# Blackgaurd/pathtracer-cpp

Hardware: AMD Instinct MI355X
Metric: Mray/s (all bounces) + achieved HBM GB/s, Cornell 1024² 10k spp depth-5 (higher is better)
Workload: dtype f32

## Files before the change

### include/pt_hip_debug.h

```cpp
#ifndef PT_HIP_DEBUG_H
#define PT_HIP_DEBUG_H

#include "pt_hip.h"

#ifdef __cplusplus
extern "C" {
#endif

int pt_debug_math(int device, int which, const float* in, int n, float* out);
int pt_debug_sweep(int device, int which, uint32_t lo_bits, uint32_t hi_bits, uint64_t* mismatches,
                   uint32_t* first_bad);
int pt_debug_rgb8(int device, const float* linear_rgb, int32_t res_x, int32_t res_y, float gamma, uint8_t* rgb8);
int pt_debug_rccl_failover(int32_t n_devices, int32_t fail_step, int64_t* out);
int pt_debug_wide_verify(const pt_scene* scene, int32_t width);
int pt_debug_pack_hash(const pt_scene* scene, uint64_t* hash);
int pt_rtc_check(const pt_scene* scene, char* src_out, size_t cap);
int pt_debug_rtc_start(const pt_scene* scene);
int64_t pt_debug_rtc_cache(int32_t op);

int pt_debug_ctx_flags(const pt_ctx* ctx, int32_t out[5]);
int pt_debug_ctx_plan(const pt_ctx* ctx, int64_t out[24]);
int pt_debug_walk_placement(int32_t num_nodes, int32_t num_tris, int32_t tree_depth, int32_t tri_f4,
                            int32_t rec_rows, uint64_t lds_usable, int32_t out[4]);
int pt_debug_scene_dark(const pt_scene* scene);
int pt_debug_emit_reject(const float* box6, const float* org, const float* dir, int64_t n, uint8_t* out);
int pt_debug_emit_slab_reject(const float* box6, const float* org, const float* inv, int64_t n, uint8_t* out);
int pt_debug_emit_box(const pt_scene* scene, float out[6]);
int pt_debug_ctx_emit_reject(const pt_ctx* ctx, int32_t* on, float box[6], uint64_t* early);
int pt_debug_ray_stack(int32_t which, int32_t count, int32_t n, int32_t reserve, int32_t flag);
int pt_debug_flat_lds(int32_t num_tris, int32_t box_tab_bytes, int32_t pair_queue, int32_t rec_size, uint32_t out[10]);
int64_t pt_debug_counter(int32_t which);

#ifdef __cplusplus
}
#endif
#endif
```

### pathtracer-cpp_amd/csrc/pt_kernel.hip

```cpp
#include <hip/hip_runtime.h>

#include <stdint.h>
#include <stdio.h>
#include <stdlib.h>
#include <string.h>

#include <algorithm>
#include <chrono>
#include <future>
#include <map>
#include <memory>
#include <mutex>
#include <string>
#include <thread>
#include <vector>

#include <atomic>

#include "pt_grad.h"
#include "pt_hip_debug.h"
#include "pt_launch.h"
#include "pt_moments.h"
#include "pt_nee_grad.h"
#include "pt_rtc.h"
// ... 176 lines not shown

__global__ void pt_math_kernel(int which, const float* __restrict__ in, float* __restrict__ out, int n) {
    const int i = blockIdx.x * blockDim.x + threadIdx.x;
    if (i >= n) return;
    if (which == 0) {
        out[i] = acosf_ref(in[i]);
    } else if (which == 1) {
        float sv, cv;
        sincosf_ref(in[i], sv, cv);
        out[2 * i] = sv;
        out[2 * i + 1] = cv;
    } else if (which == 2) {
        const float* a = in + 9 * (size_t)i;
        Lcg g{__float_as_uint(a[0])};
        const int type = __float_as_int(a[1]);
        const v3 dd{a[3], a[4], a[5]}, nn{a[6], a[7], a[8]};
        v3 r;
        if (type == PT_MAT_SPECULAR) specular_dir(g, dd, nn, a[2], kMaxSpecularIters, r);
        else r = hemisphere_dir(g, nn);
        out[4 * i] = r.x;
        out[4 * i + 1] = r.y;
        out[4 * i + 2] = r.z;
        out[4 * i + 3] = __uint_as_float(g.s);
    }
}

__global__ void pt_sweep_kernel(int which, uint32_t lo, unsigned long long n, unsigned long long* bad,
                                uint32_t* first) {
    unsigned long long nb = 0;
    uint32_t fb = 0xffffffffu;
    const unsigned long long stride = (unsigned long long)gridDim.x * blockDim.x;
    for (unsigned long long i = (unsigned long long)blockIdx.x * blockDim.x + threadIdx.x; i < n; i += stride) {
        const uint32_t bits = lo + (uint32_t)i;
        const float x = __uint_as_float(bits);
        if (x != x) continue;
        bool same;
        if (which == 0) {
            same = __float_as_uint(rcp_exact(x)) == __float_as_uint(1.0f / x);
        } else if (which == 1) {
            same = __float_as_uint(sqrt_exact(x)) == __float_as_uint(__builtin_sqrtf(x));
        } else if (which == 4) {
            const float ax = __builtin_fabsf(x);
            if (!(ax >= 0x1p-60f && ax <= 0x1p60f)) continue;
            const uint32_t hsh = pt_mix32(bits * 0x9e3779b9u + 0x7f4a7c15u);
            const uint32_t e = (bits & 1u) ? 67u + (hsh >> 23) % 121u : 127u + (hsh >> 23) % 11u;
            const float b = __uint_as_float((e << 23) | (hsh & 0x7fffffu));
// ... 2290 lines not shown
    const EmitBox e = scene_emit_box(ps, scene_dark(ps));
    for (int a = 0; a < 3; a++) out[a] = e.lo[a], out[3 + a] = e.hi[a];
    return e.on ? 1 : 0;
}

int pt_debug_emit_reject(const float* box6, const float* org, const float* dir, int64_t n, uint8_t* out) {
    if (!box6 || !org || !dir || !out || n < 0) return set_error(PT_E_ARG, "pt_debug_emit_reject: bad argument");
    for (int64_t i = 0; i < n; i++) {
        const float *b = box6 + 6 * i, *o = org + 3 * i, *d = dir + 3 * i;
        out[i] = emit_reject(v3{b[0], b[1], b[2]}, v3{b[3], b[4], b[5]}, v3{o[0], o[1], o[2]}, v3{d[0], d[1], d[2]}) ? 1 : 0;
    }
    return PT_OK;
}

int pt_debug_emit_slab_reject(const float* box6, const float* org, const float* inv, int64_t n, uint8_t* out) {
    if (!box6 || !org || !inv || !out || n < 0) return set_error(PT_E_ARG, "pt_debug_emit_slab_reject: bad argument");
    for (int64_t i = 0; i < n; i++) {
        const float *b = box6 + 6 * i, *o = org + 3 * i, *v = inv + 3 * i;
        out[i] = emit_slab_reject(v3{b[0], b[1], b[2]}, v3{b[3], b[4], b[5]}, v3{o[0], o[1], o[2]}, v3{v[0], v[1], v[2]}) ? 1 : 0;
    }
    return PT_OK;
}

int pt_debug_ray_stack(int32_t which, int32_t count, int32_t n, int32_t reserve, int32_t flag) {
    switch (which) {
        case 0: return ray_stack_generate(count, n, reserve, flag != 0) ? 1 : 0;
        case 1: return ray_stack_filled(count, n);
        case 2: return ray_stack_dry(count, n) ? 1 : 0;
        case 3: return ray_stack_slot(count, n);
        case 4: return ray_stack_taken(count, n);
        case 5: return ray_stack_done(flag != 0, count, n != 0) ? 1 : 0;
    }
    return set_error(PT_E_ARG, "pt_debug_ray_stack: which = %d", which);
}

int pt_debug_flat_lds(int32_t num_tris, int32_t box_tab_bytes, int32_t pair_queue, int32_t rec_size, uint32_t out[10]) {
    if (!out || num_tris < 0 || box_tab_bytes < 0 || pair_queue < 0 || rec_size < 0)
        return set_error(PT_E_ARG, "pt_debug_flat_lds: bad argument");
    const FlatLds l = flat_lds_layout(3u * (unsigned)num_tris, 2u * (unsigned)num_tris, (unsigned)box_tab_bytes,
                                      (unsigned)pair_queue, (unsigned)rec_size);
    const uint32_t v[10] = {l.tris, l.mats, l.next_ray, l.best, l.next_at, l.boxtab, l.queues, l.rec_tri, l.rec_cos, l.bytes};
    memcpy(out, v, sizeof(v));
    return PT_OK;
}

int pt_debug_ctx_plan(const pt_ctx* c, int64_t out[24]) {
// ... 67 lines not shown
```

### pathtracer-cpp_amd/csrc/pt_math.h

```cpp
#pragma once

#if !defined(__HIPCC_RTC__)
#include <stdint.h>
#endif

#if defined(__HIPCC__)
#define PT_HD __host__ __device__ __forceinline__
#else
#define PT_HD inline
#endif

namespace pt {

PT_HD uint32_t f2u(float f) { return __builtin_bit_cast(uint32_t, f); }
PT_HD float u2f(uint32_t u) { return __builtin_bit_cast(float, u); }

struct v3 {
    float x, y, z;
};
PT_HD v3 mk(float x, float y, float z) { return v3{x, y, z}; }
PT_HD v3 add(v3 a, v3 b) { return v3{a.x + b.x, a.y + b.y, a.z + b.z}; }
PT_HD v3 sub(v3 a, v3 b) { return v3{a.x - b.x, a.y - b.y, a.z - b.z}; }
PT_HD v3 mul(v3 a, v3 b) { return v3{a.x * b.x, a.y * b.y, a.z * b.z}; }
PT_HD v3 scale(v3 a, float s) { return v3{a.x * s, a.y * s, a.z * s}; }
// ... 65 lines not shown
    if (__builtin_expect(out, 0)) return __builtin_sqrtf(x);
    return sqrt_fixup(x);
#endif
#else
    return __builtin_sqrtf(x);
#endif
}

template <bool kUnit = false>
PT_HD v3 rcp3_exact(v3 d, bool live = true) {
#if defined(__HIP_DEVICE_COMPILE__) && PT_WAVE_GUARD
    const float ax = __builtin_fabsf(d.x), ay = __builtin_fabsf(d.y), az = __builtin_fabsf(d.z);
    bool out = !(__builtin_fminf(__builtin_fminf(ax, ay), az) >= 0x1p-126f);
    if (!kUnit) out = out || !(__builtin_fmaxf(__builtin_fmaxf(ax, ay), az) <= 0x1p126f);
    v3 r{rcp_newton(d.x), rcp_newton(d.y), rcp_newton(d.z)};
    if (__builtin_expect(wave_any(live && out), 0)) r = v3{1.0f / d.x, 1.0f / d.y, 1.0f / d.z};
    return r;
#else
    (void)live;
    return v3{rcp_exact(d.x), rcp_exact(d.y), rcp_exact(d.z)};
#endif
}

PT_HD v3 normalize(v3 a) {
    float len = sqrt_exact(dot(a, a));
    return v3{a.x / len, a.y / len, a.z / len};
}

PT_HD float div_by_rcp(float a, float b, float y) {
#if defined(__HIP_DEVICE_COMPILE__)
    const float q0 = a * y;
    return __builtin_fmaf(__builtin_fmaf(-b, q0, a), y, q0);
#else
    (void)y;
    return a / b;
#endif
}

PT_HD v3 normalize_fast(v3 a) {
#if defined(__HIP_DEVICE_COMPILE__) && PT_WAVE_GUARD
    const float l2 = dot(a, a);
    const float mn = __builtin_fminf(__builtin_fminf(__builtin_fabsf(a.x), __builtin_fabsf(a.y)), __builtin_fabsf(a.z));
    const bool out = !(l2 >= 0x1p-100f && l2 <= 0x1p100f && mn >= 0x1p-60f);
    const float lf = sqrt_fixup(l2), y = rcp_newton(lf);
    v3 r{div_by_rcp(a.x, lf, y), div_by_rcp(a.y, lf, y), div_by_rcp(a.z, lf, y)};
    if (__builtin_expect(wave_any(out), 0)) {
// ... 48 lines not shown
    float t1x = (lb.x - o.x) * inv.x, t1y = (lb.y - o.y) * inv.y, t1z = (lb.z - o.z) * inv.z;
    float t2x = (rt.x - o.x) * inv.x, t2y = (rt.y - o.y) * inv.y, t2z = (rt.z - o.z) * inv.z;
    float tmax = __builtin_fminf(__builtin_fminf(__builtin_fmaxf(t1x, t2x), __builtin_fmaxf(t1y, t2y)),
                                 __builtin_fmaxf(t1z, t2z));
    float tmin = __builtin_fmaxf(__builtin_fmaxf(__builtin_fminf(t1x, t2x), __builtin_fminf(t1y, t2y)),
                                 __builtin_fminf(t1z, t2z));
    return __builtin_fmaxf(tmin, 0.0f) <= tmax;
}

PT_HD bool all_finite(v3 a) {
    return __builtin_fabsf(a.x) < __builtin_inff() && __builtin_fabsf(a.y) < __builtin_inff() &&
           __builtin_fabsf(a.z) < __builtin_inff();
}

PT_HD int emit_reject_axis(float lo, float hi, float o, float d) {
    return (int)(__builtin_fabsf(d) < 2.0f) & (((int)(o < lo) & (int)(d < 0.0f)) | ((int)(o > hi) & (int)(d > 0.0f)));
}
PT_HD bool emit_reject(v3 elb, v3 ert, v3 o, v3 d) {
    return (emit_reject_axis(elb.x, ert.x, o.x, d.x) | emit_reject_axis(elb.y, ert.y, o.y, d.y) |
            emit_reject_axis(elb.z, ert.z, o.z, d.z)) != 0;
}

PT_HD bool finite_nonzero(float x) { return ((int)(__builtin_fabsf(x) < __builtin_inff()) & (int)(x != 0.0f)) != 0; }
PT_HD bool emit_slab_reject_nonempty(v3 elb, v3 ert, v3 o, v3 inv, bool behind_only = false) {
    const int guard = (int)finite_nonzero(inv.x) & (int)finite_nonzero(inv.y) & (int)finite_nonzero(inv.z) &
                      (int)(__builtin_fabsf(o.x) < __builtin_inff()) & (int)(__builtin_fabsf(o.y) < __builtin_inff()) &
                      (int)(__builtin_fabsf(o.z) < __builtin_inff());
    const float t1x = (elb.x - o.x) * inv.x, t1y = (elb.y - o.y) * inv.y, t1z = (elb.z - o.z) * inv.z;
    const float t2x = (ert.x - o.x) * inv.x, t2y = (ert.y - o.y) * inv.y, t2z = (ert.z - o.z) * inv.z;
    const float tmax = __builtin_fminf(__builtin_fminf(__builtin_fmaxf(t1x, t2x), __builtin_fmaxf(t1y, t2y)),
                                       __builtin_fmaxf(t1z, t2z));
    const float tmin = __builtin_fmaxf(__builtin_fmaxf(__builtin_fminf(t1x, t2x), __builtin_fminf(t1y, t2y)),
                                       __builtin_fminf(t1z, t2z));
    return (guard & ((int)(tmax < 0.0f) | ((int)!behind_only & (int)(tmin > tmax)))) != 0;
}
PT_HD bool emit_box_empty(v3 elb, v3 ert) {
    return ((int)(elb.x > ert.x) | (int)(elb.y > ert.y) | (int)(elb.z > ert.z)) != 0;
}
PT_HD bool emit_slab_reject(v3 elb, v3 ert, v3 o, v3 inv) {
    return emit_box_empty(elb, ert) ? true : emit_slab_reject_nonempty(elb, ert, o, inv);
}

PT_HD bool tri_hit(v3 v1, v3 e1, v3 e2, v3 o, v3 d, float& t) {
    v3 h = cross(d, e2);
    float a = dot(e1, h);
    if (__builtin_fabsf(a) < 0x1.0c6f7cp-20f) return false;
    float f = rcp_exact(a);
    v3 s = sub(o, v1);
    float u = f * dot(s, h);
    if (u < 0.0f || u > 1.0f) return false;
    v3 q = cross(s, e1);
    float v = f * dot(d, q);
    if (v < 0.0f || u + v > 1.0f) return false;
    t = f * dot(e2, q);
    return t > 0.0f;
}

PT_HD bool tri_hit_nb(v3 v1, v3 e1, v3 e2, v3 o, v3 d, float& t) {
    v3 h = cross(d, e2);
    float a = dot(e1, h);
    const bool ok = !(__builtin_fabsf(a) < 0x1.0c6f7cp-20f);
#if defined(__HIP_DEVICE_COMPILE__)
    const float r = __builtin_amdgcn_rcpf(a);
// ... 232 lines not shown
```

### pathtracer-cpp_amd/csrc/pt_rtc.hip

```cpp
#include <hip/hip_runtime.h>
#include <hip/hiprtc.h>

#include <dlfcn.h>
#include <errno.h>
#include <fcntl.h>
#include <link.h>
#include <signal.h>
#include <spawn.h>
#include <stdint.h>
#include <stdio.h>
#include <stdlib.h>
#include <string.h>
#include <sys/socket.h>
#include <sys/stat.h>
#include <sys/wait.h>
#include <unistd.h>

#include <algorithm>
#include <atomic>
#include <chrono>
#include <fstream>
#include <future>
#include <limits>
#include <map>
// ... 210 lines not shown
            chain += std::string("        ") + w + " = shl1_add_bit(" + w + ", __builtin_amdgcn_ballot_w64(b" +
                     std::to_string(u) + "));\n";
        }
        acc = "#if KBOX\n        uint32_t lo, hi;\n" + chain + "#else\n" + acc + "#endif\n";
    }
    acc += "        const unsigned long long m = ((unsigned long long)hi << 32) | lo;\n";
    const bool single = leaves_single(leaves, n);
    const bool sign = tri_fast;
    std::string tabs = "{";
    for (size_t u = 0; u < box_tab.size(); u++) tabs += (u ? ", " : "") + std::to_string(box_tab[u]) + "u";
    tabs += box_tab.empty() ? "0u}" : "}";
    std::string rej = "    using EmitRej = NoEmitReject;\n";
    if (emit.on)
        rej = "    struct EmitRej {\n        static constexpr bool kCompiled = true;\n"
              "        __device__ __forceinline__ static bool on() { return true; }\n"
              "        __device__ __forceinline__ static bool rejected(v3 o, v3 d) {\n"
              "            return emit_reject(v3{" + litf(emit.lo[0]) + ", " + litf(emit.lo[1]) + ", " + litf(emit.lo[2]) +
              "}, v3{" + litf(emit.hi[0]) + ", " + litf(emit.hi[1]) + ", " + litf(emit.hi[2]) + "}, o, d);\n"
              "        }\n"
              "        static constexpr bool kSlab = !PT_EMIT_SIGN_ONLY;\n"
              "        __device__ __forceinline__ static bool rejected_slab(v3 o, v3, v3 inv) {\n"
              "            return emit_slab_reject(v3{" + litf(emit.lo[0]) + ", " + litf(emit.lo[1]) + ", " + litf(emit.lo[2]) +
              "}, v3{" + litf(emit.hi[0]) + ", " + litf(emit.hi[1]) + ", " + litf(emit.hi[2]) + "}, o, inv);\n"
              "        }\n    };\n";
    return std::string("#ifndef PT_FLAT_SIGN_MASK\n#define PT_FLAT_SIGN_MASK 0\n#endif\n#define KSIGN (PT_FLAT_SIGN_MASK && ") +
           (sign ? "1" : "0") + ")\n" + "#define KBOX " + (nbox > 0 ? "(!KSIGN)" : "0") + "\n" +
           "namespace pt {\nstruct SceneBoxMask {\n    static constexpr bool kSignMask = KSIGN;\n"
           "    static constexpr bool kBoxPairs = KBOX;\n    static constexpr bool kCamInvGen = PT_CAM_INV == 2;\n"
           "    static constexpr bool kRayStack = PT_RAY_STACK != 0;\n"
           "    static constexpr int kBoxes = " + std::to_string(nbox) +
           ";\n    static constexpr uint16_t kBoxTab[" + std::to_string(std::max<size_t>(1, box_tab.size())) + "] = " + tabs +
           ";\n    static constexpr bool kMask32 = " +
           (n <= 32 ? "true" : "false") + ";\n    static constexpr bool kSingleTri = " + (single ? "true" : "false") +
           ";\n    static constexpr bool kSpecular = " + (specular ? "true" : "false") +
           ";\n    static constexpr bool kTriFast = " + (tri_fast ? "true" : "false") +
           ";\n    static constexpr bool kAlbedoX2 = " + (albedo_x2 ? "true" : "false") +
           ";\n    static constexpr bool kDarkKnown = true;\n    static constexpr bool kDark = " + (dark ? "true" : "false") +
           ";\n    static constexpr bool kBaked = PT_KCONST != 0;\n    static constexpr int kNumTri4 = " +
           std::to_string(baked.num_tri4) + ", kNumMat4 = " + std::to_string(baked.num_mat4) +
           ", kBoxTabBytes = " + std::to_string(baked.box_tab_bytes) + ", kThetaLanes = " + std::to_string(baked.theta_lanes) +
           ";\n    static constexpr bool kPairs = " + (baked.pairs ? "true" : "false") +
           ";\n" + rej + "    __device__ __forceinline__ static unsigned long long "
           "mask(const TraceArgs&, v3 o, v3 inv) {\n" +
           body + tests + acc + "        return m;\n    }\n};\n}  // namespace pt\n";
}

struct RtcCache {
    std::mutex mu;
    std::map<std::string, RtcFuture> code;
    std::map<std::pair<int, std::string>, hipFunction_t> funcs;
    std::set<std::string> refused;
};
// ... 560 lines not shown
```

### pathtracer-cpp_amd/csrc/pt_trace.h

```cpp
#pragma once

#include "pt_hip.h"
#include "pt_math.h"
#include "pt_flatlds.h"
#include "pt_raystack.h"

namespace pt {

constexpr int kBlock = 256;
constexpr int kWave = 64;
static_assert(kRaySlots == kWave, "one prefetched camera ray per lane (pt_raystack.h)");
constexpr int kMaxSpecularIters = 1 << 16;
#ifndef PT_CHUNK
#define PT_CHUNK 1024
#endif
constexpr int kChunk = PT_CHUNK;
static_assert(kChunk >= kWave, "a work-pool refill must cover one claim of every lane of a wave");
constexpr int kMaxFlatLeaves = 64;

#ifndef PT_WAVES
#define PT_WAVES 7
#endif

#ifdef PT_STAMPS
// ... 301 lines not shown
constexpr int kEmitSlab = 1, kEmitSignOnly = 2, kEmitSlabEmpty = 3;
#ifndef PT_EMIT_SIGN_ONLY
#define PT_EMIT_SIGN_ONLY 0
#endif
struct KernargEmitSlabReject : KernargEmitReject {
    static constexpr bool kSlab = true;
    __device__ __forceinline__ static bool rejected_slab(v3 o, v3, v3 inv) {
        const auto* K = kernarg_args();
        const int mode = K->emit_on;
        if (mode == kEmitSlabEmpty) return true;
        return emit_slab_reject_nonempty(v3{K->emit_lo_x, K->emit_lo_y, K->emit_lo_z},
                                         v3{K->emit_hi_x, K->emit_hi_y, K->emit_hi_z}, o, inv, mode == kEmitSignOnly);
    }
};
template <typename Rej, typename = void>
struct RejSlab {
    static constexpr bool value = false;
};
template <typename Rej>
struct RejSlab<Rej, decltype((void)Rej::kSlab)> {
    static constexpr bool value = Rej::kCompiled && Rej::kSlab;
};

struct NodeBox {
    v3 lb, rt;
    int a, b;
};

__device__ __forceinline__ NodeBox load_node(const float4* __restrict__ nodes, int n) {
    const float4 p = nodes[2 * n], q = nodes[2 * n + 1];
    return NodeBox{v3{p.x, p.y, p.z}, v3{p.w, q.x, q.y}, __float_as_int(q.z), __float_as_int(q.w)};
}

template <bool kFiniteInv>
__device__ __forceinline__ bool box_hit(v3 lb, v3 rt, v3 o, v3 inv) {
    return kFiniteInv ? slab_hit_finite(lb, rt, o, inv) : slab_hit(lb, rt, o, inv);
}

template <bool kFiniteInv, typename NodePtr, typename TriPtr>
__device__ __forceinline__ int intersect_tree(NodePtr nodes, TriPtr tris, int* __restrict__ stk, int tid, v3 o,
                                              v3 d, v3 inv, float& t_out) {
    int hit = -1;
    float t = 1e30f;
    int sp = 0;
    const NodeBox root = load_node(nodes, 0);
    int ca = root.a, cb = root.b;
// ... 1138 lines not shown

#ifndef PT_CAM_KERNARG
#define PT_CAM_KERNARG 1
#endif
__device__ __forceinline__ void camera_ray(const TraceArgs& A, int q, int s, Lcg& g, v3& o, v3& d) {
    const auto* K = PT_CAM_KERNARG ? kernarg_args() : nullptr;
    const TraceArgs& C = PT_CAM_KERNARG ? *(const TraceArgs*)K : A;
    const int r = (int)fdiv((uint32_t)q, C.div_w);
    const int px = q - r * C.W;
    const int py = part_row(C, r);
    g.s = pt_sample_seed((uint32_t)(py * C.W + px), (uint32_t)s, C.seed);
    const float jy = g.next01();
    const float jx = g.next01();
    const float cx = ((float)px + jx) * C.cell - C.half_vres_x;
    const float cy = ((float)py + jy) * C.cell - C.half_vres_y;
    d = normalize_fast(v3{cx * C.col0_x + cy * C.col0_y + C.cz_col0, cx * C.col1_x + cy * C.col1_y + C.cz_col1,
                     cx * C.col2_x + cy * C.col2_y + C.cz_col2});
    o = v3{C.pos_x, C.pos_y, C.pos_z};
}

constexpr int kShadeGo = 0, kShadeEnd = 1, kShadeEndEarly = 2;

template <bool kSpecular = true, typename RecT = int, bool kIds = false, typename Rej = NoEmitReject,
          typename KC = ArgConsts>
__device__ __forceinline__ int shade_inv(const TraceArgs& A, const float4* __restrict__ mats,
                                          const float4* __restrict__ tris, RecT* __restrict__ rec_tri,
                                          float* __restrict__ rec_cos, int tid, int hit, float t, Lcg& g, v3& o,
                                          v3& d, v3& inv, int& k, v3& L, const KC& kc = KC()) {
    L = v3{0.0f, 0.0f, 0.0f};
    if (hit < 0) return kShadeEnd;
#ifdef PT_EXP_DUP_SHADE
    {
        int h2 = hit;
        asm volatile("" : "+v"(h2));
        const float4 tn2 = kIds ? tris[h2] : tris[3 * h2 + 2];
        const int row2 = kIds ? __float_as_int(tn2.w) : h2;
        const float4 m02 = mats[2 * row2], m12 = mats[2 * row2 + 1];
        v3 n2 = kIds ? v3{tn2.x, tn2.y, tn2.z} : v3{tn2.y, tn2.z, tn2.w};
        if (!(dot(n2, d) < 0.0f)) n2 = neg(n2);
        const v3 hp2 = add(o, scale(d, t));
        asm volatile("" ::"v"(m02.x), "v"(m12.x), "v"(hp2.x), "v"(hp2.y), "v"(hp2.z), "v"(n2.x), "v"(n2.y), "v"(n2.z));
    }
#endif
    float4 tn;
    int row = hit;
    if constexpr (kIds) {
        tn = tris[hit];
        row = __float_as_int(tn.w);
    }
    const float4 m0 = mats[2 * row], m1 = mats[2 * row + 1];
    const int type = __float_as_int(m0.x);
// ... 48 lines not shown
            const v3 x = hemisphere_dir(g2, n);
            asm volatile("" ::"v"(x.x), "v"(x.y), "v"(x.z));
        }
#endif
#endif
#if defined(PT_EXP_COHERENT_DIR) || defined(PT_EXP_OCTANT_DIR)
        {
            const v3 w = v3{__int_as_float(__builtin_amdgcn_readfirstlane(__float_as_int(nd.x))),
                            __int_as_float(__builtin_amdgcn_readfirstlane(__float_as_int(nd.y))),
                            __int_as_float(__builtin_amdgcn_readfirstlane(__float_as_int(nd.z)))};
#ifdef PT_EXP_COHERENT_DIR
            nd = dot(w, n) < 0.0f ? neg(w) : w;
#else
            const v3 c = v3{__builtin_copysignf(nd.x, w.x), __builtin_copysignf(nd.y, w.y), __builtin_copysignf(nd.z, w.z)};
            if (dot(c, n) >= 0.0f) nd = c;
#endif
        }
#endif
    }
    rec_tri[k * kBlock + tid] = (RecT)row;
    rec_cos[k * kBlock + tid] = dot(n, nd);
    o = add(hp, scale(n, 1e-4f));
    d = nd;
    if constexpr (RejSlab<Rej>::value) inv = rcp3_exact<!kSpecular>(d);
    if constexpr (Rej::kCompiled) {
        if (Rej::on()) {
            bool rej;
            if constexpr (RejSlab<Rej>::value) rej = Rej::rejected_slab(o, d, inv);
            else rej = Rej::rejected(o, d);
            const bool early = ((int)(k + 2 >= depth) & (int)rej) != 0;
            k += early ? 0 : 1;
            return early ? kShadeEndEarly : kShadeGo;
        }
    }
    k++;
    return kShadeGo;
}

template <bool kSpecular = true, typename RecT = int, bool kIds = false, typename Rej = NoEmitReject>
__device__ __forceinline__ int shade(const TraceArgs& A, const float4* __restrict__ mats,
                                      const float4* __restrict__ tris, RecT* __restrict__ rec_tri,
                                      float* __restrict__ rec_cos, int tid, int hit, float t, Lcg& g, v3& o, v3& d,
                                      int& k, v3& L) {
    static_assert(!RejSlab<Rej>::value, "a policy with the slab rule carries inv: shade_inv");
    v3 unused{0.0f, 0.0f, 0.0f};
    return shade_inv<kSpecular, RecT, kIds, Rej>(A, mats, tris, rec_tri, rec_cos, tid, hit, t, g, o, d, unused, k, L);
}

__device__ __forceinline__ uint32_t slab_index(const TraceArgs& A, int s, int q) {
    return (uint32_t)(s - A.s_begin) * (uint32_t)A.npix + (uint32_t)q;
}
// ... 79 lines not shown
    if (unwind && fl) {
        if (kc.flags_pm()) {
            const uint32_t sm = fdiv(at, A.div_npix), q = at - sm * (uint32_t)A.npix;
            atomicOr(fl + flag_word(sm, q, (uint32_t)A.npix), 1u << (sm & 31u));
        } else {
            atomicOr(fl + (at >> 5), 1u << (at & 31u));
        }
    }
}

__device__ __forceinline__ void count_rays(const TraceArgs& A, int lane, uint32_t n_rays) {
    unsigned long long r = n_rays;
    for (int off = 32; off > 0; off >>= 1) r += __shfl_down(r, off);
    if (lane == 0) atomicAdd(A.ctr + 1, r);
}

__device__ __forceinline__ void count_rays_wave(const TraceArgs& A, int lane, unsigned long long n_rays) {
    if (lane == 0) atomicAdd(A.ctr + 1, n_rays);
}

#ifndef PT_COUNT_EARLY
#define PT_COUNT_EARLY 0
#endif
__device__ __forceinline__ void count_early_wave(const TraceArgs& A, int lane, unsigned long long n_early) {
    if (PT_COUNT_EARLY && lane == 0 && n_early) atomicAdd(A.ctr + 4, n_early);
}

#ifndef PT_FRESH_TID
#define PT_FRESH_TID 1
#endif
#ifndef PT_CAM_INV
#define PT_CAM_INV 2
#endif
#ifndef PT_RAY_STACK
#define PT_RAY_STACK 1
#endif
#ifndef PT_RAY_RESERVE
#define PT_RAY_RESERVE (-1)
#endif
__device__ __forceinline__ int fresh_tid() {
    int t = (int)threadIdx.x;
    if (PT_FRESH_TID) asm volatile("" : "+v"(t));
    return t;
}

struct FlatRecs {
    uint16_t* tri;
    float* cos;
// ... 27 lines not shown
    for (int i = tid; i < kc.num_tri4(A); i += kBlock) s_tris[i] = A.tris[i];
    for (int i = tid; i < kc.num_mat4(A); i += kBlock) {
        float4 m = A.mats[i];
        if (BoxMask::kAlbedoX2 && !(i & 1)) m = make_float4(m.x, 2.0f * m.y, 2.0f * m.z, 2.0f * m.w);
        s_mats[i] = m;
    }
    __syncthreads();
    const float4* __restrict__ mats = s_mats;
    const float4* __restrict__ tris = s_tris;
    uint16_t* wq = queues + __builtin_amdgcn_readfirstlane(tid >> 6) * kc.pair_queue(A);

    bool alive = true;
    bool active = false;
    bool has_next = false;
    int count = 0;
    bool dry = false;
    uint32_t at = 0;
    Lcg g{0};
    v3 o{0, 0, 0}, d{0, 0, 0};
    constexpr bool kCarry = RejSlab<typename BoxMask::EmitRej>::value;
    v3 inv{0, 0, 0};
    constexpr bool kGenInv = kCarry && BoxMask::kCamInvGen;
    v3 next_inv{0, 0, 0};
    int k = 0;
    unsigned long long n_rays = 0;
    unsigned long long n_early = 0;
    Pool pool = pool_start(A);
#ifdef PT_STAMPS
    uint64_t stamp_acc[kStampSections] = {};
#endif

    while (true) {
        PT_STAMP(st_a)
        auto generate = [&](uint32_t item) {
            const uint32_t blk = fdiv(item, A.div_npix);
            Lcg gn{0};
            v3 on, nd;
            camera_ray(A, (int)(item - blk * (uint32_t)A.npix), A.s_begin + (int)blk, gn, on, nd);
#ifdef PT_EXP_DUP_CAMF
            {
                uint32_t it2 = item;
                asm volatile("" : "+v"(it2));
                Lcg g2{0};
                v3 o2, d2;
                camera_ray(A, (int)(it2 - blk * (uint32_t)A.npix), A.s_begin + (int)blk, g2, o2, d2);
                asm volatile("" ::"v"(d2.x), "v"(d2.y), "v"(d2.z), "v"(g2.s));
            }
#endif
            next_ray[fresh_tid()] = make_float4(nd.x, nd.y, nd.z, __uint_as_float(gn.s));
            next_at[fresh_tid()] = item;
            if constexpr (kGenInv) next_inv = rcp3_exact(nd);
        };
        if constexpr (BoxMask::kRayStack) {
            const unsigned long long need = __ballot(!active);
            const int n_need = (int)__popcll(need);
            if (ray_stack_generate(count, n_need, PT_RAY_RESERVE >= 0 ? PT_RAY_RESERVE : A.ray_reserve, dry)) {
                const bool want = lane >= count;
                bool got = true;
                uint32_t item = 0;
                claim_item(A, lane, want, pool, got, item);
                if (want && got) generate(item);
                const int n_got = (int)__popcll(__ballot(want && got));
#ifdef PT_STAMPS
                stamp_acc[11] += 1;
                stamp_acc[12] += (uint32_t)n_got;
#endif
                dry = ray_stack_dry(count, n_got);
                count = ray_stack_filled(count, n_got);
                wave_lds_sync();
            }
            if (n_need > 0 && count > 0) {
                const int rank = (int)__builtin_amdgcn_mbcnt_hi((uint32_t)(need >> 32),
                                                                __builtin_amdgcn_mbcnt_lo((uint32_t)need, 0u));
                const int slot = ray_stack_slot(count, rank);
                const bool take = !active && slot >= 0;
                v3 ti{0, 0, 0};
                if constexpr (kGenInv)
                    ti = v3{lane_float(slot << 2, next_inv.x), lane_float(slot << 2, next_inv.y),
                            lane_float(slot << 2, next_inv.z)};
                if (take) {
                    const int t0 = (fresh_tid() & ~(kWave - 1)) + slot;
                    const float4 nr = next_ray[t0];
                    at = next_at[t0];
                    g.s = __float_as_uint(nr.w);
                    d = v3{nr.x, nr.y, nr.z};
                    if constexpr (kGenInv) inv = ti;
                    else if constexpr (kCarry) inv = rcp3_exact(d);
                    o = v3{A.pos_x, A.pos_y, A.pos_z};
                    k = 0;
                    active = true;
                }
                count = ray_stack_taken(count, n_need);
            }
            if (ray_stack_done(__any(active), count, dry)) break;
        } else {
            const bool want = alive && !has_next;
            const int n_want = (int)__popcll(__ballot(want));
            if (n_want > 0 && (n_want >= A.regen_thresh || !__any(active || has_next))) {
                uint32_t item = 0;
                claim_item(A, lane, want, pool, alive, item);
                if (want && alive) {
                    generate(item);
                    has_next = true;
                }
#ifdef PT_STAMPS
                stamp_acc[11] += 1;
                stamp_acc[12] += (uint32_t)__popcll(__ballot(want && alive));
#endif
            }
            if (!active && has_next) {
                const int t0 = fresh_tid();
                const float4 nr = next_ray[t0];
                at = next_at[t0];
                g.s = __float_as_uint(nr.w);
                d = v3{nr.x, nr.y, nr.z};
                if constexpr (kGenInv) inv = next_inv;
                else if constexpr (kCarry) inv = rcp3_exact(d);
                o = v3{A.pos_x, A.pos_y, A.pos_z};
                k = 0;
                active = true;
                has_next = false;
            }
            if (!__any(active)) break;
        }
        PT_STAMP(st_b)

        float t = 0.0f;
        int hit = -1;
        const bool tr = active && kc.depth(A) > 0;
        if (kc.depth(A) > 0) n_rays += (unsigned long long)__popcll(__ballot(tr));
        if constexpr (!kCarry) inv = rcp3_exact(d, tr);
        const bool forced = A.force_exact_slab == 1 || (A.force_exact_slab == 2 && ((tid >> 6) & 1));
        const bool fast = !forced && __all(!tr || (BoxMask::kSignMask ? bounded_ray(o, inv) : all_finite(inv)));
        if (fast && kc.pairs_on(A)) {
            if (PT_PRIO_MASK) __builtin_amdgcn_s_setprio(PT_PRIO_MASK);
            unsigned long long mask = BoxMask::mask(A, o, inv);
#ifdef PT_EXP_DUP_MASK
            {
                v3 o2 = o;
                asm volatile("" : "+v"(o2.x));
                const unsigned long long m2 = BoxMask::mask(A, o2, inv);
                asm volatile("" ::"v"((uint32_t)m2), "v"((uint32_t)(m2 >> 32)));
            }
#endif
            if (PT_PRIO_MASK) __builtin_amdgcn_s_setprio(0);
            if (!tr) mask = 0ull;
            PT_STAMP(st_b2)
            PT_STAMP_ADD(1, st_b, st_b2)
#ifdef PT_STAMPS
            {
                const uint32_t pc = (uint32_t)__popcll(mask);
                const uint32_t tot = (uint32_t)__builtin_amdgcn_readlane((int)wave_incl_scan(pc), 63);
                int mx = (int)pc;
                for (int off = 32; off > 0; off >>= 1) mx = max(mx, __shfl_xor(mx, off));
                stamp_acc[7] += 1;
                stamp_acc[8] += tot;
                stamp_acc[9] += (tot + 63) / 64;
                stamp_acc[10] += (uint32_t)mx;
            }
#endif
#ifdef PT_EXP_NO_PAIRS
            hit = mask ? __builtin_ctzll(mask) : -1;
            t = 1.0f;
#else
            if (PT_PRIO_PAIRS) __builtin_amdgcn_s_setprio(PT_PRIO_PAIRS);
            hit = intersect_flat_pairs<BoxMask>(A, mask, kc.leaves(A), tris, wq, best, fresh_tid(), lane, o, d, t, boxtab, kc);
            if (PT_PRIO_PAIRS) __builtin_amdgcn_s_setprio(0);
#endif
            PT_STAMP(st_b3)
            PT_STAMP_ADD(2, st_b2, st_b3)
        } else if (tr) {
            if (fast && !kc.pairs_on(A)) hit = intersect_flat<BoxMask>(A, kc.leaves(A), tris, o, d, inv, t, boxtab);
            else hit = intersect_tree<false>(kc.nodes(A), tris, kc.exact_stack(A), tid, o, d, inv, t);
        }
        PT_STAMP(st_c)

        int sh = kShadeGo;
        v3 L{0.0f, 0.0f, 0.0f};
        if (PT_PRIO_SHADE) __builtin_amdgcn_s_setprio(PT_PRIO_SHADE);
        if (active) {
            const FlatRecs R = flat_records<BoxMask>(lds4, kc);
            sh = shade_inv<BoxMask::kSpecular, uint16_t, false, typename BoxMask::EmitRej>(
                A, mats, tris, R.tri, R.cos, fresh_tid(), hit, t, g, o, d, inv, k, L, kc);
        }
        if (PT_PRIO_SHADE) __builtin_amdgcn_s_setprio(0);
        const bool end = sh != kShadeGo;
        if constexpr (BoxMask::EmitRej::kCompiled) {
            const unsigned long long ne = (unsigned long long)__popcll(__ballot(sh == kShadeEndEarly));
            n_rays += ne;
            if (PT_COUNT_EARLY) n_early += ne;
        }
        PT_STAMP(st_d)
        if (end) {
            if (PT_PRIO_FOLD) __builtin_amdgcn_s_setprio(PT_PRIO_FOLD);
            const FlatRecs R = flat_records<BoxMask>(lds4, kc);
            finish_path<uint16_t, BoxMask::kAlbedoX2, BoxMask::kDarkKnown, BoxMask::kDark>(A, mats, R.tri, R.cos,
                                                                                        fresh_tid(), k, L, at, kc);
            if (PT_PRIO_FOLD) __builtin_amdgcn_s_setprio(0);
            active = false;
        }
        PT_STAMP(st_e)
        PT_STAMP_ADD(0, st_a, st_b)
        PT_STAMP_ADD(5, st_b, st_c)
        PT_STAMP_ADD(3, st_c, st_d)
        PT_STAMP_ADD(4, st_d, st_e)
    }
#ifdef PT_STAMPS
    if (lane == 0 && A.stamps) {
        for (int i = 0; i < kStampSections; i++)
            if (i != 6) atomicAdd(A.stamps + i, (unsigned long long)stamp_acc[i]);
        atomicAdd(A.stamps + 6, 1ull);
    }
#endif
    drain_accumulate(A, lane);
    count_rays_wave(A, lane, n_rays);
    count_early_wave(A, lane, n_early);
}

#ifndef PT_FLAT_ONLY
template <bool kLdsScene>
__device__ __forceinline__ void trace_body(const TraceArgs& A) {
    extern __shared__ float4 lds4[];
// ... 342 lines not shown
```

Before: 82450.

## Check ray-direction domain once per bounce and track active lanes as a wave mask

When the reciprocal direction is computed, a domain check now records a per-path mark bit in the path index. The per-bounce wave-wide all_finite vote over inv is skipped unless some lane carries that mark, and the emitter slab reject reuses the precomputed finiteness flag instead of recomputing it. Separately, when the ray stack is used, the active-lane predicate is held as a scalar 64-bit wave mask and turned back into per-lane booleans with inverse_ballot, replacing repeated ballots and __any votes. This trims vector compares and cross-lane votes from the hot loop, at the cost of extra masking logic and of reusing a high bit of the path index as a flag.

```diff
diff --git a/include/pt_hip_debug.h b/include/pt_hip_debug.h
--- a/include/pt_hip_debug.h
+++ b/include/pt_hip_debug.h
@@ -25,6 +25,9 @@
 int pt_debug_scene_dark(const pt_scene* scene);
 int pt_debug_emit_reject(const float* box6, const float* org, const float* dir, int64_t n, uint8_t* out);
 int pt_debug_emit_slab_reject(const float* box6, const float* org, const float* inv, int64_t n, uint8_t* out);
+int pt_debug_domain_once(int device, const float* box6, const float* org, const float* dir, int64_t n, int unit,
+                         uint8_t* out, float* inv3);
+int pt_debug_hemisphere_dir(const uint32_t* lcg, const float* nrm, int64_t n, float* dir3);
 int pt_debug_emit_box(const pt_scene* scene, float out[6]);
 int pt_debug_ctx_emit_reject(const pt_ctx* ctx, int32_t* on, float box[6], uint64_t* early);
 int pt_debug_ray_stack(int32_t which, int32_t count, int32_t n, int32_t reserve, int32_t flag);
diff --git a/pathtracer-cpp_amd/csrc/pt_kernel.hip b/pathtracer-cpp_amd/csrc/pt_kernel.hip
--- a/pathtracer-cpp_amd/csrc/pt_kernel.hip
+++ b/pathtracer-cpp_amd/csrc/pt_kernel.hip
@@ -222,6 +222,41 @@
         out[4 * i + 1] = r.y;
         out[4 * i + 2] = r.z;
         out[4 * i + 3] = __uint_as_float(g.s);
+    }
+}
+
+template <bool kUnit>
+PT_HD void domain_once_probe(v3 elb, v3 ert, v3 o, v3 d, uint8_t* r, float* inv3) {
+    const float ax = __builtin_fabsf(d.x), ay = __builtin_fabsf(d.y), az = __builtin_fabsf(d.z);
+    bool in = __builtin_fminf(__builtin_fminf(ax, ay), az) >= 0x1p-126f;
+    if (!kUnit) in = in && __builtin_fmaxf(__builtin_fmaxf(ax, ay), az) <= 0x1p126f;
+    bool fell;
+    const v3 inv = rcp3_exact_v<kUnit>(d, fell);
+    const bool inv_ok = fell ? finite_nonzero3(inv) : true;
+    r[0] = in;
+    r[1] = finite_nonzero3(inv);
+    r[2] = all_finite(inv);
+    r[3] = !fell;
+    r[4] = emit_slab_reject(elb, ert, o, inv);
+    r[5] = emit_slab_reject_given(elb, ert, o, inv, inv_ok);
+    inv3[0] = inv.x;
+    inv3[1] = inv.y;
+    inv3[2] = inv.z;
+}
+__global__ void pt_domain_once_kernel(const float* box6, const float* org, const float* dir, int n, int unit,
+                                      uint8_t* out, float* inv3) {
+    const v3 elb{box6[0], box6[1], box6[2]}, ert{box6[3], box6[4], box6[5]};
+    for (int base = 0; base < n; base += (int)blockDim.x) {
+        const int i = base + (int)threadIdx.x, j = i < n ? i : n - 1;
+        const v3 o{org[3 * j], org[3 * j + 1], org[3 * j + 2]}, d{dir[3 * j], dir[3 * j + 1], dir[3 * j + 2]};
+        uint8_t r[6];
+        float v[3];
+        if (unit) domain_once_probe<true>(elb, ert, o, d, r, v);
+        else domain_once_probe<false>(elb, ert, o, d, r, v);
+        if (i < n) {
+            for (int c = 0; c < 6; c++) out[6 * i + c] = r[c];
+            for (int c = 0; c < 3; c++) inv3[3 * i + c] = v[c];
+        }
     }
 }
 
@@ -2558,6 +2593,56 @@
     return PT_OK;
 }
 
+int pt_debug_domain_once(int device, const float* box6, const float* org, const float* dir, int64_t n, int unit,
+                         uint8_t* out, float* inv3) {
+    if (!box6 || !org || !dir || !out || !inv3 || n < 1 || n > (1 << 20))
+        return set_error(PT_E_ARG, "pt_debug_domain_once: bad argument");
+    if (device < 0) {
+        const v3 elb{box6[0], box6[1], box6[2]}, ert{box6[3], box6[4], box6[5]};
+        for (int64_t i = 0; i < n; i++) {
+            const v3 o{org[3 * i], org[3 * i + 1], org[3 * i + 2]}, d{dir[3 * i], dir[3 * i + 1], dir[3 * i + 2]};
+            if (unit) domain_once_probe<true>(elb, ert, o, d, out + 6 * i, inv3 + 3 * i);
+            else domain_once_probe<false>(elb, ert, o, d, out + 6 * i, inv3 + 3 * i);
+        }
+        return PT_OK;
+    }
+    HIP_TRY(hipSetDevice(device));
+    const size_t fb = (size_t)n * 3 * sizeof(float);
+    float* dbuf = nullptr;
+    uint8_t* dout = nullptr;
+    HIP_TRY(hipMalloc((void**)&dbuf, 6 * sizeof(float) + 3 * fb));
+    if (hipMalloc((void**)&dout, (size_t)n * 6) != hipSuccess) {
+        (void)hipFree(dbuf);
+        return set_error(PT_E_HIP, "hipMalloc failed");
+    }
+    float *dorg = dbuf + 6, *ddir = dorg + 3 * n, *dinv = ddir + 3 * n;
+    hipError_t e = hipMemcpy(dbuf, box6, 6 * sizeof(float), hipMemcpyHostToDevice);
+    if (e == hipSuccess) e = hipMemcpy(dorg, org, fb, hipMemcpyHostToDevice);
+    if (e == hipSuccess) e = hipMemcpy(ddir, dir, fb, hipMemcpyHostToDevice);
+    if (e == hipSuccess) {
+        hipLaunchKernelGGL(pt_domain_once_kernel, dim3(1), dim3(256), 0, 0, dbuf, dorg, ddir, (int)n, unit, dout, dinv);
+        e = hipGetLastError();
+    }
+    if (e == hipSuccess) e = hipMemcpy(out, dout, (size_t)n * 6, hipMemcpyDeviceToHost);
+    if (e == hipSuccess) e = hipMemcpy(inv3, dinv, fb, hipMemcpyDeviceToHost);
+    (void)hipFree(dbuf);
+    (void)hipFree(dout);
+    if (e != hipSuccess) return set_error(PT_E_HIP, "pt_debug_domain_once: %s", hipGetErrorString(e));
+    return PT_OK;
+}
+
+int pt_debug_hemisphere_dir(const uint32_t* lcg, const float* nrm, int64_t n, float* dir3) {
+    if (!lcg || !nrm || !dir3 || n < 0) return set_error(PT_E_ARG, "pt_debug_hemisphere_dir: bad argument");
+    for (int64_t i = 0; i < n; i++) {
+        Lcg g{lcg[i]};
+        const v3 r = hemisphere_dir(g, v3{nrm[3 * i], nrm[3 * i + 1], nrm[3 * i + 2]});
+        dir3[3 * i] = r.x;
+        dir3[3 * i + 1] = r.y;
+        dir3[3 * i + 2] = r.z;
+    }
+    return PT_OK;
+}
+
 int pt_debug_ray_stack(int32_t which, int32_t count, int32_t n, int32_t reserve, int32_t flag) {
     switch (which) {
         case 0: return ray_stack_generate(count, n, reserve, flag != 0) ? 1 : 0;
diff --git a/pathtracer-cpp_amd/csrc/pt_math.h b/pathtracer-cpp_amd/csrc/pt_math.h
--- a/pathtracer-cpp_amd/csrc/pt_math.h
+++ b/pathtracer-cpp_amd/csrc/pt_math.h
@@ -111,6 +111,22 @@
 #endif
 }
 
+template <bool kUnit>
+PT_HD v3 rcp3_exact_v(v3 d, bool& fell) {
+    const float ax = __builtin_fabsf(d.x), ay = __builtin_fabsf(d.y), az = __builtin_fabsf(d.z);
+    bool out = !(__builtin_fminf(__builtin_fminf(ax, ay), az) >= 0x1p-126f);
+    if (!kUnit) out = out || !((ax + ay) + az <= 0x1p126f);
+#if defined(__HIP_DEVICE_COMPILE__) && PT_WAVE_GUARD
+    v3 r{rcp_newton(d.x), rcp_newton(d.y), rcp_newton(d.z)};
+    fell = wave_any(out);
+    if (__builtin_expect(fell, 0)) r = v3{1.0f / d.x, 1.0f / d.y, 1.0f / d.z};
+    return r;
+#else
+    fell = out;
+    return v3{rcp_exact(d.x), rcp_exact(d.y), rcp_exact(d.z)};
+#endif
+}
+
 PT_HD v3 normalize(v3 a) {
     float len = sqrt_exact(dot(a, a));
     return v3{a.x / len, a.y / len, a.z / len};
@@ -205,9 +221,11 @@
 }
 
 PT_HD bool finite_nonzero(float x) { return ((int)(__builtin_fabsf(x) < __builtin_inff()) & (int)(x != 0.0f)) != 0; }
-PT_HD bool emit_slab_reject_nonempty(v3 elb, v3 ert, v3 o, v3 inv, bool behind_only = false) {
-    const int guard = (int)finite_nonzero(inv.x) & (int)finite_nonzero(inv.y) & (int)finite_nonzero(inv.z) &
-                      (int)(__builtin_fabsf(o.x) < __builtin_inff()) & (int)(__builtin_fabsf(o.y) < __builtin_inff()) &
+PT_HD bool finite_nonzero3(v3 a) {
+    return ((int)finite_nonzero(a.x) & (int)finite_nonzero(a.y) & (int)finite_nonzero(a.z)) != 0;
+}
+PT_HD bool emit_slab_reject_core(v3 elb, v3 ert, v3 o, v3 inv, bool behind_only, bool inv_ok) {
+    const int guard = (int)inv_ok & (int)(__builtin_fabsf(o.x) < __builtin_inff()) & (int)(__builtin_fabsf(o.y) < __builtin_inff()) &
                       (int)(__builtin_fabsf(o.z) < __builtin_inff());
     const float t1x = (elb.x - o.x) * inv.x, t1y = (elb.y - o.y) * inv.y, t1z = (elb.z - o.z) * inv.z;
     const float t2x = (ert.x - o.x) * inv.x, t2y = (ert.y - o.y) * inv.y, t2z = (ert.z - o.z) * inv.z;
@@ -217,11 +235,17 @@
                                        __builtin_fminf(t1z, t2z));
     return (guard & ((int)(tmax < 0.0f) | ((int)!behind_only & (int)(tmin > tmax)))) != 0;
 }
+PT_HD bool emit_slab_reject_nonempty(v3 elb, v3 ert, v3 o, v3 inv, bool behind_only = false) {
+    return emit_slab_reject_core(elb, ert, o, inv, behind_only, finite_nonzero3(inv));
+}
 PT_HD bool emit_box_empty(v3 elb, v3 ert) {
     return ((int)(elb.x > ert.x) | (int)(elb.y > ert.y) | (int)(elb.z > ert.z)) != 0;
 }
 PT_HD bool emit_slab_reject(v3 elb, v3 ert, v3 o, v3 inv) {
     return emit_box_empty(elb, ert) ? true : emit_slab_reject_nonempty(elb, ert, o, inv);
+}
+PT_HD bool emit_slab_reject_given(v3 elb, v3 ert, v3 o, v3 inv, bool inv_ok) {
+    return emit_box_empty(elb, ert) ? true : emit_slab_reject_core(elb, ert, o, inv, false, inv_ok);
 }
 
 PT_HD bool tri_hit(v3 v1, v3 e1, v3 e2, v3 o, v3 d, float& t) {
diff --git a/pathtracer-cpp_amd/csrc/pt_rtc.hip b/pathtracer-cpp_amd/csrc/pt_rtc.hip
--- a/pathtracer-cpp_amd/csrc/pt_rtc.hip
+++ b/pathtracer-cpp_amd/csrc/pt_rtc.hip
@@ -256,12 +256,17 @@
               "        __device__ __forceinline__ static bool rejected_slab(v3 o, v3, v3 inv) {\n"
               "            return emit_slab_reject(v3{" + litf(emit.lo[0]) + ", " + litf(emit.lo[1]) + ", " + litf(emit.lo[2]) +
               "}, v3{" + litf(emit.hi[0]) + ", " + litf(emit.hi[1]) + ", " + litf(emit.hi[2]) + "}, o, inv);\n"
+              "        }\n"
+              "        __device__ __forceinline__ static bool rejected_slab_given(v3 o, v3, v3 inv, bool inv_ok) {\n"
+              "            return emit_slab_reject_given(v3{" + litf(emit.lo[0]) + ", " + litf(emit.lo[1]) + ", " + litf(emit.lo[2]) +
+              "}, v3{" + litf(emit.hi[0]) + ", " + litf(emit.hi[1]) + ", " + litf(emit.hi[2]) + "}, o, inv, inv_ok);\n"
               "        }\n    };\n";
     return std::string("#ifndef PT_FLAT_SIGN_MASK\n#define PT_FLAT_SIGN_MASK 0\n#endif\n#define KSIGN (PT_FLAT_SIGN_MASK && ") +
            (sign ? "1" : "0") + ")\n" + "#define KBOX " + (nbox > 0 ? "(!KSIGN)" : "0") + "\n" +
            "namespace pt {\nstruct SceneBoxMask {\n    static constexpr bool kSignMask = KSIGN;\n"
            "    static constexpr bool kBoxPairs = KBOX;\n    static constexpr bool kCamInvGen = PT_CAM_INV == 2;\n"
            "    static constexpr bool kRayStack = PT_RAY_STACK != 0;\n"
+           "    static constexpr bool kDomOnce = PT_DOMAIN_ONCE != 0;\n"
            "    static constexpr int kBoxes = " + std::to_string(nbox) +
            ";\n    static constexpr uint16_t kBoxTab[" + std::to_string(std::max<size_t>(1, box_tab.size())) + "] = " + tabs +
            ";\n    static constexpr bool kMask32 = " +
diff --git a/pathtracer-cpp_amd/csrc/pt_trace.h b/pathtracer-cpp_amd/csrc/pt_trace.h
--- a/pathtracer-cpp_amd/csrc/pt_trace.h
+++ b/pathtracer-cpp_amd/csrc/pt_trace.h
@@ -347,6 +347,25 @@
     static constexpr bool value = Rej::kCompiled && Rej::kSlab;
 };
 
+#ifndef PT_DOMAIN_ONCE
+#define PT_DOMAIN_ONCE 1
+#endif
+constexpr uint32_t kDomMark = 0x80000000u;
+#if defined(__has_builtin) && __has_builtin(__builtin_amdgcn_inverse_ballot_w64)
+__device__ __forceinline__ bool pt_lane_of_mask(unsigned long long m) { return __builtin_amdgcn_inverse_ballot_w64(m); }
+#else
+extern "C" __device__ bool pt_lane_of_mask(unsigned long long) __asm("llvm.amdgcn.inverse.ballot.i64");
+#endif
+template <typename M, typename = void>
+struct DomOnce {
+    static constexpr bool value = false, kMasks = false;
+};
+template <typename M>
+struct DomOnce<M, decltype((void)M::kDomOnce)> {
+    static constexpr bool value = M::kDomOnce && !M::kSignMask && RejSlab<typename M::EmitRej>::value;
+    static constexpr bool kMasks = M::kDomOnce;
+};
+
 struct NodeBox {
     v3 lb, rt;
     int a, b;
@@ -1531,11 +1550,12 @@
 constexpr int kShadeGo = 0, kShadeEnd = 1, kShadeEndEarly = 2;
 
 template <bool kSpecular = true, typename RecT = int, bool kIds = false, typename Rej = NoEmitReject,
-          typename KC = ArgConsts>
+          typename KC = ArgConsts, bool kDom = false>
 __device__ __forceinline__ int shade_inv(const TraceArgs& A, const float4* __restrict__ mats,
                                           const float4* __restrict__ tris, RecT* __restrict__ rec_tri,
                                           float* __restrict__ rec_cos, int tid, int hit, float t, Lcg& g, v3& o,
-                                          v3& d, v3& inv, int& k, v3& L, const KC& kc = KC()) {
+                                          v3& d, v3& inv, int& k, v3& L, const KC& kc = KC(),
+                                          uint32_t* dom_at = nullptr) {
     L = v3{0.0f, 0.0f, 0.0f};
     if (hit < 0) return kShadeEnd;
 #ifdef PT_EXP_DUP_SHADE
@@ -1630,11 +1650,21 @@
     rec_cos[k * kBlock + tid] = dot(n, nd);
     o = add(hp, scale(n, 1e-4f));
     d = nd;
-    if constexpr (RejSlab<Rej>::value) inv = rcp3_exact<!kSpecular>(d);
+    bool fell = true;
+    bool inv_ok = true;
+    if constexpr (kDom) {
+        static_assert(RejSlab<Rej>::value, "the domain policy goes with the carried inv");
+        inv = rcp3_exact_v<!kSpecular>(d, fell);
+        if (__builtin_expect(fell, 0)) {
+            *dom_at |= kDomMark;
+            inv_ok = finite_nonzero3(inv);
+        }
+    } else if constexpr (RejSlab<Rej>::value) inv = rcp3_exact<!kSpecular>(d);
     if constexpr (Rej::kCompiled) {
         if (Rej::on()) {
             bool rej;
-            if constexpr (RejSlab<Rej>::value) rej = Rej::rejected_slab(o, d, inv);
+            if constexpr (kDom) rej = Rej::rejected_slab_given(o, d, inv, inv_ok);
+            else if constexpr (RejSlab<Rej>::value) rej = Rej::rejected_slab(o, d, inv);
             else rej = Rej::rejected(o, d);
             const bool early = ((int)(k + 2 >= depth) & (int)rej) != 0;
             k += early ? 0 : 1;
@@ -1760,8 +1790,11 @@
 #ifndef PT_COUNT_EARLY
 #define PT_COUNT_EARLY 0
 #endif
+#ifndef PT_COUNT_DOM
+#define PT_COUNT_DOM 0
+#endif
 __device__ __forceinline__ void count_early_wave(const TraceArgs& A, int lane, unsigned long long n_early) {
-    if (PT_COUNT_EARLY && lane == 0 && n_early) atomicAdd(A.ctr + 4, n_early);
+    if ((PT_COUNT_EARLY || PT_COUNT_DOM) && lane == 0 && n_early) atomicAdd(A.ctr + 4, n_early);
 }
 
 #ifndef PT_FRESH_TID
@@ -1835,6 +1868,9 @@
     v3 inv{0, 0, 0};
     constexpr bool kGenInv = kCarry && BoxMask::kCamInvGen;
     v3 next_inv{0, 0, 0};
+    constexpr bool kDom = DomOnce<BoxMask>::value;
+    constexpr bool kActMask = DomOnce<BoxMask>::kMasks && BoxMask::kRayStack;
+    unsigned long long act = 0;
     int k = 0;
     unsigned long long n_rays = 0;
     unsigned long long n_early = 0;
@@ -1862,10 +1898,23 @@
 #endif
             next_ray[fresh_tid()] = make_float4(nd.x, nd.y, nd.z, __uint_as_float(gn.s));
             next_at[fresh_tid()] = item;
-            if constexpr (kGenInv) next_inv = rcp3_exact(nd);
+            if constexpr (kGenInv && kDom) {
+                bool fell;
+                next_inv = rcp3_exact_v<false>(nd, fell);
+                if (__builtin_expect(fell, 0)) next_at[fresh_tid()] = item | kDomMark;
+            } else if constexpr (kGenInv) next_inv = rcp3_exact(nd);
+        };
+        auto start_inv = [&]() {
+            if constexpr (kDom) {
+                bool fell;
+                inv = rcp3_exact_v<false>(d, fell);
+                if (__builtin_expect(fell, 0)) at |= kDomMark;
+            } else inv = rcp3_exact(d);
         };
         if constexpr (BoxMask::kRayStack) {
-            const unsigned long long need = __ballot(!active);
+            unsigned long long need;
+            if constexpr (kActMask) need = ~act;
+            else need = __ballot(!active);
             const int n_need = (int)__popcll(need);
             if (ray_stack_generate(count, n_need, PT_RAY_RESERVE >= 0 ? PT_RAY_RESERVE : A.ray_reserve, dry)) {
                 const bool want = lane >= count;
@@ -1886,7 +1935,14 @@
                 const int rank = (int)__builtin_amdgcn_mbcnt_hi((uint32_t)(need >> 32),
                                                                 __builtin_amdgcn_mbcnt_lo((uint32_t)need, 0u));
                 const int slot = ray_stack_slot(count, rank);
-                const bool take = !active && slot >= 0;
+                bool take;
+                if constexpr (kActMask) {
+                    const unsigned long long takers = __ballot(slot >= 0) & need;
+                    take = pt_lane_of_mask(takers);
+                    act |= takers;
+                } else {
+                    take = !active && slot >= 0;
+                }
                 v3 ti{0, 0, 0};
                 if constexpr (kGenInv)
                     ti = v3{lane_float(slot << 2, next_inv.x), lane_float(slot << 2, next_inv.y),
@@ -1898,14 +1954,17 @@
                     g.s = __float_as_uint(nr.w);
                     d = v3{nr.x, nr.y, nr.z};
                     if constexpr (kGenInv) inv = ti;
-                    else if constexpr (kCarry) inv = rcp3_exact(d);
+                    else if constexpr (kCarry) start_inv();
                     o = v3{A.pos_x, A.pos_y, A.pos_z};
                     k = 0;
-                    active = true;
+                    if constexpr (!kActMask) active = true;
                 }
                 count = ray_stack_taken(count, n_need);
             }
-            if (ray_stack_done(__any(active), count, dry)) break;
+            bool any_path;
+            if constexpr (kActMask) any_path = act != 0ull;
+            else any_path = __any(active);
+            if (ray_stack_done(any_path, count, dry)) break;
         } else {
             const bool want = alive && !has_next;
             const int n_want = (int)__popcll(__ballot(want));
@@ -1928,7 +1987,7 @@
                 g.s = __float_as_uint(nr.w);
                 d = v3{nr.x, nr.y, nr.z};
                 if constexpr (kGenInv) inv = next_inv;
-                else if constexpr (kCarry) inv = rcp3_exact(d);
+                else if constexpr (kCarry) start_inv();
                 o = v3{A.pos_x, A.pos_y, A.pos_z};
                 k = 0;
                 active = true;
@@ -1940,11 +1999,35 @@
 
         float t = 0.0f;
         int hit = -1;
-        const bool tr = active && kc.depth(A) > 0;
-        if (kc.depth(A) > 0) n_rays += (unsigned long long)__popcll(__ballot(tr));
+        unsigned long long trm = 0ull;
+        bool tr;
+        if constexpr (kActMask) {
+            trm = kc.depth(A) > 0 ? act : 0ull;
+            tr = pt_lane_of_mask(trm);
+            n_rays += (unsigned long long)__popcll(trm);
+        } else {
+            tr = active && kc.depth(A) > 0;
+            if (kc.depth(A) > 0) n_rays += (unsigned long long)__popcll(__ballot(tr));
+        }
         if constexpr (!kCarry) inv = rcp3_exact(d, tr);
         const bool forced = A.force_exact_slab == 1 || (A.force_exact_slab == 2 && ((tid >> 6) & 1));
-        const bool fast = !forced && __all(!tr || (BoxMask::kSignMask ? bounded_ray(o, inv) : all_finite(inv)));
+        bool fast;
+        if constexpr (kDom) {
+            bool fin_all = true;
+            unsigned long long marked;
+            if constexpr (kActMask) marked = __ballot((int)at < 0) & trm;
+            else marked = __ballot(tr && (int)at < 0);
+            if (__builtin_expect(marked != 0ull, 0)) {
+                const bool fin = all_finite(inv);
+                if (fin) at &= ~kDomMark;
+                if constexpr (kActMask) fin_all = (trm & ~__ballot(fin)) == 0ull;
+                else fin_all = __all(!tr || fin);
+                if (PT_COUNT_DOM) n_early += (unsigned long long)__popcll(marked);
+            }
+            fast = !forced && fin_all;
+        } else {
+            fast = !forced && __all(!tr || (BoxMask::kSignMask ? bounded_ray(o, inv) : all_finite(inv)));
+        }
         if (fast && kc.pairs_on(A)) {
             if (PT_PRIO_MASK) __builtin_amdgcn_s_setprio(PT_PRIO_MASK);
             unsigned long long mask = BoxMask::mask(A, o, inv);
@@ -1991,13 +2074,23 @@
         int sh = kShadeGo;
         v3 L{0.0f, 0.0f, 0.0f};
         if (PT_PRIO_SHADE) __builtin_amdgcn_s_setprio(PT_PRIO_SHADE);
-        if (active) {
+        bool shading;
+        if constexpr (kActMask) shading = pt_lane_of_mask(act);
+        else shading = active;
+        if (shading) {
             const FlatRecs R = flat_records<BoxMask>(lds4, kc);
-            sh = shade_inv<BoxMask::kSpecular, uint16_t, false, typename BoxMask::EmitRej>(
-                A, mats, tris, R.tri, R.cos, fresh_tid(), hit, t, g, o, d, inv, k, L, kc);
+            sh = shade_inv<BoxMask::kSpecular, uint16_t, false, typename BoxMask::EmitRej, KC, kDom>(
+                A, mats, tris, R.tri, R.cos, fresh_tid(), hit, t, g, o, d, inv, k, L, kc, &at);
         }
         if (PT_PRIO_SHADE) __builtin_amdgcn_s_setprio(0);
-        const bool end = sh != kShadeGo;
+        bool end;
+        if constexpr (kActMask) {
+            const unsigned long long endm = __ballot(sh != kShadeGo);
+            end = pt_lane_of_mask(endm);
+            act &= ~endm;
+        } else {
+            end = sh != kShadeGo;
+        }
         if constexpr (BoxMask::EmitRej::kCompiled) {
             const unsigned long long ne = (unsigned long long)__popcll(__ballot(sh == kShadeEndEarly));
             n_rays += ne;
@@ -2008,9 +2101,10 @@
             if (PT_PRIO_FOLD) __builtin_amdgcn_s_setprio(PT_PRIO_FOLD);
             const FlatRecs R = flat_records<BoxMask>(lds4, kc);
             finish_path<uint16_t, BoxMask::kAlbedoX2, BoxMask::kDarkKnown, BoxMask::kDark>(A, mats, R.tri, R.cos,
-                                                                                        fresh_tid(), k, L, at, kc);
+                                                                                        fresh_tid(), k, L,
+                                                                                        kDom ? at & ~kDomMark : at, kc);
             if (PT_PRIO_FOLD) __builtin_amdgcn_s_setprio(0);
-            active = false;
+            if constexpr (!kActMask) active = false;
         }
         PT_STAMP(st_e)
         PT_STAMP_ADD(0, st_a, st_b)
```

Result: faster. 84010, median of 6 (+1.9%).
